# MoHawastaken/Gaussian-Process-Regression

Hardware: AMD Instinct MI355X
Metric: GPR predict-step achieved fp64 TFLOP/s (kernel fill + Cholesky + solves + mean/variance), n x n sqexp (higher is better)
Workload: dtype f64; 1 GPU; c4: n=65536 d=8 sqrexp GPR fit+predict, n*=65536 (reference test-grid rule), noise=0.1; n=65536, d=8, n_star=65536, kernel=sqrexp, parallelism=1-D block-cyclic 512-column panels over 1 GPU(s), test points sliced

## Files before the change

### gaussian-process-regression_amd/_native.py

```python
from __future__ import annotations

import ctypes as C
import os
import threading

import numpy as np

_HERE = os.path.dirname(os.path.abspath(__file__))
LIB_PATH = os.path.join(_HERE, "lib", "libgprc_native" + os.environ.get("GPRC_LIB_SUFFIX", "") + ".so")

CONSTANT, LINEAR, POLYNOMIAL, SQREXP, GAMMAEXP, RATQUAD, SQREXP_ARD, MATERN32, MATERN52, MATERN32_ARD, MATERN52_ARD = range(11)
ARD_KERNELS = (SQREXP_ARD, MATERN32_ARD, MATERN52_ARD)

OK = 0
GPC_REFERENCE_STOP = 1
ERR_ARG, ERR_HIP, ERR_NOMEM, ERR_NOT_PD, ERR_DIVERGED, ERR_MAXITER, ERR_NO_DEVICE = -1, -2, -3, -4, -5, -6, -7


class GprcError(RuntimeError):

    def __init__(self, status: int, message: str):
        super().__init__(f"gprc native error {status}: {message}")
        self.status = status
        self.message = message


class NotPositiveDefinite(ArithmeticError):

    def __init__(self, info: int):
        super().__init__(f"the leading minor of order {info} is not positive definite")
        self.info = info


_dp = C.POINTER(C.c_double)
_i64 = C.c_int64
_vp = C.c_void_p

PROTOTYPES = {
    "gprc_abi_version": (C.c_int, []),
    "gprc_last_error": (C.c_char_p, []),
    "gprc_device_count": (C.c_int, [C.POINTER(C.c_int)]),
    "gprc_ctx_create": (C.c_int, [C.c_int, _vp, C.POINTER(_vp)]),
    "gprc_ctx_destroy": (C.c_int, [_vp]),
    "gprc_ctx_synchronize": (C.c_int, [_vp]),
    "gprc_ctx_trim": (C.c_int, [_vp]),
    "gprc_kernel_matrix": (C.c_int, [_vp, C.c_int, _dp, C.c_int, _vp, _i64, _i64, _vp, _i64, _vp, _i64]),
    "gprc_kernel_colwise": (C.c_int, [_vp, C.c_int, _dp, C.c_int, _vp, _vp, _i64, _i64, _vp]),
    "gprc_gpr_fit": (C.c_int, [_vp, C.c_int, _dp, C.c_int, _vp, _i64, _i64, _vp, C.c_double, C.POINTER(_vp)]),
    "gprc_gpr_fit_retry": (C.c_int, [_vp, C.c_int, _dp, C.c_int, _vp, _i64, _i64, _vp, C.c_double, C.POINTER(_vp),
                                     C.POINTER(C.c_double), C.POINTER(C.c_int)]),
    "gprc_gpr_log_marginal": (C.c_int, [_vp, C.c_int, _dp, C.c_int, _vp, _i64, _i64, _vp, C.c_double, C.POINTER(C.c_double)]),
    "gprc_fit_gradient": (C.c_int, [_vp, C.c_int, _dp, C.c_int, _vp, _i64, _i64, _vp, _dp]),
    "gprc_gpr_logp_grad": (C.c_int, [_vp, C.c_int, _dp, C.c_int, _vp, _i64, _i64, _vp, C.c_double, C.POINTER(C.c_double), _dp]),
    "gprc_gpr_batch_logp_grad": (C.c_int, [_vp, C.c_int, _i64, _vp, C.c_int, _i64, _vp, _vp, _i64, _i64, _i64, _vp, _i64, _vp, _vp, _vp, _vp, _vp]),
    "gprc_gpr_batch_fit": (C.c_int, [_vp, C.c_int, _i64, _vp, C.c_int, _i64, _vp, _vp, _i64, _i64, _i64, _vp, _i64, _vp, C.POINTER(_vp), _vp, _vp]),
    "gprc_gpr_batch_predict": (C.c_int, [_vp, _vp, _i64, _i64, _vp, _vp, _vp, _i64]),
    "gprc_gpr_batch_predict_grad": (C.c_int, [_vp, _vp, _i64, _i64, _vp, _vp, _vp, _i64, _vp, _vp, _i64]),
    "gprc_gpr_batch_loo": (C.c_int, [_vp, _vp, _vp, _vp, _i64, _vp]),
    "gprc_gpr_batch_get_alpha": (C.c_int, [_vp, _vp]),
    "gprc_batch_model_dims": (C.c_int, [_vp, C.POINTER(_i64), C.POINTER(_i64), C.POINTER(_i64)]),
    "gprc_batch_model_free": (C.c_int, [_vp]),
    "gprc_dev_knn": (C.c_int, [_vp, _vp, _i64, _i64, _vp, _i64, _vp, _i64, _vp, _vp, _i64]),
    "gprc_lgpr_create": (C.c_int, [_vp, C.c_int, _dp, C.c_int, _vp, _i64, _i64, _vp, C.c_double, _i64, C.POINTER(_vp)]),
    "gprc_lgpr_set_params": (C.c_int, [_vp, _dp, C.c_int, C.c_double]),
    "gprc_lgpr_predict": (C.c_int, [_vp, _vp, _i64, _vp, _vp, _vp]),
    "gprc_lgpr_neighbours": (C.c_int, [_vp, _vp, _i64, _vp, _vp, _i64]),
    "gprc_lgpr_dims": (C.c_int, [_vp, C.POINTER(_i64), C.POINTER(_i64), C.POINTER(_i64)]),
    "gprc_lgpr_free": (C.c_int, [_vp]),
    "gprc_gpr_loo": (C.c_int, [_vp, _vp, _vp, _vp, C.POINTER(C.c_double)]),
    "gprc_gpr_loo_grad": (C.c_int, [_vp, C.c_int, _dp, C.c_int, _vp, _i64, _i64, _vp, C.c_double, C.POINTER(C.c_double), _dp]),
    "gprc_gpr_predict": (C.c_int, [_vp, _vp, _i64, C.c_int, _vp, _vp]),
    "gprc_gpr_predict_grad": (C.c_int, [_vp, _vp, _i64, _vp, _vp, _vp, _vp]),
    "gprc_gpr_extend": (C.c_int, [_vp, _vp, _i64, _vp]),
    "gprc_model_dims": (C.c_int, [_vp, C.POINTER(_i64), C.POINTER(_i64)]),
    "gprc_model_get_L": (C.c_int, [_vp, _vp, _i64]),
    "gprc_gpr_get_alpha": (C.c_int, [_vp, _vp]),
    "gprc_gpr_get_logp": (C.c_int, [_vp, C.POINTER(C.c_double)]),
    "gprc_gpr_get_noise": (C.c_int, [_vp, C.POINTER(C.c_double)]),
    "gprc_model_free": (C.c_int, [_vp]),
    "gprc_gpc_fit": (C.c_int, [_vp, C.c_int, _dp, C.c_int, _vp, _i64, _i64, _vp, C.c_double, C.c_int, C.c_int, C.POINTER(_vp),
                               C.POINTER(C.c_int)]),
    "gprc_gpc_predict_latent": (C.c_int, [_vp, _vp, _i64, _vp, _vp]),
    "gprc_gpc_predict_class": (C.c_int, [_vp, _vp, _i64, _vp]),
    "gprc_class_probability": (C.c_int, [_vp, _vp, _vp, _i64, _vp]),
    "gprc_gpc_get_f_hat": (C.c_int, [_vp, _vp]),
    "gprc_gpc_get_logq": (C.c_int, [_vp, C.POINTER(C.c_double)]),
    "gprc_gpc_logq_grad": (C.c_int, [_vp, C.c_int, _dp, C.c_int, _vp, _i64, _i64, _vp, C.c_double, C.c_int, C.POINTER(C.c_double), _dp,
                                     C.POINTER(C.c_int)]),
    "gprc_panel_width": (_i64, []),
    "gprc_pad": (_i64, [_i64]),
    "gprc_panel_count": (_i64, [_i64]),
    "gprc_panel_offset": (_i64, [_i64, _i64]),
    "gprc_panel_elems": (_i64, [_i64, _i64]),
    "gprc_packed_size": (_i64, [_i64]),
    "gprc_winv_size": (_i64, [_i64]),
    "gprc_dev_fill_panel": (C.c_int, [_vp, C.c_int, _dp, C.c_int, _vp, _i64, _i64, _i64, C.c_double, _vp, _i64]),
    "gprc_dev_factor_panel": (C.c_int, [_vp, _vp, _i64, _i64, _vp, _vp]),
    "gprc_dev_factor_subpanel": (C.c_int, [_vp, _vp, _i64, _i64, C.c_int, C.c_int, _vp, _vp]),
    "gprc_dev_factor_all": (C.c_int, [_vp, _vp, _i64, _vp, _vp, _vp]),
    "gprc_factor_service": (C.c_int, [C.c_int]),
    "gprc_solve_inv_size": (_i64, [_i64]),
    "gprc_dev_solve_prepare": (C.c_int, [_vp, _vp, _vp, _i64, _vp, _i64, _i64]),
    "gprc_dev_update_trailing": (C.c_int, [_vp, _vp, _i64, _i64, _i64, _i64, _i64]),
    "gprc_dev_update_range": (C.c_int, [_vp, _vp, _i64, _i64, _i64, _i64, _i64, _i64]),
    "gprc_trsv_work_size": (_i64, [_i64]),
    "gprc_dev_trsv": (C.c_int, [_vp, _vp, _vp, _i64, _vp, C.c_int, _vp]),
    "gprc_dev_trsv_step": (C.c_int, [_vp, _vp, _vp, _i64, _vp, C.c_int, _i64, _vp]),
    "gprc_dev_fill_cross": (C.c_int, [_vp, C.c_int, _dp, C.c_int, _vp, _i64, _i64, _i64, _vp, _i64, _i64, _vp, _i64]),
    "gprc_rowreduce_splits": (_i64, [_i64]),
    "gprc_dev_row_reduce": (C.c_int, [_vp, _vp, _i64, _i64, _i64, _vp, _vp, _vp]),
    "gprc_dev_logp": (C.c_int, [_vp, _vp, _i64, _i64, _vp, _vp, _vp]),
    "gprc_gpr_model_from_device": (C.c_int, [_vp, C.c_int, _dp, C.c_int, _vp, _i64, _i64, _vp, _vp, _vp, _vp, C.c_double,
                                             C.c_double, C.POINTER(_vp)]),
    "gprc_mgpu_create": (C.c_int, [C.POINTER(C.c_int), C.c_int, C.c_int, C.POINTER(_vp)]),
    "gprc_mgpu_destroy": (C.c_int, [_vp]),
    "gprc_mgpu_ranks": (C.c_int, [_vp, C.POINTER(C.c_int)]),
    "gprc_mgpu_calibrate": (C.c_int, [_vp, _i64, C.c_int, C.POINTER(C.c_int), C.POINTER(C.c_double)]),
    "gprc_mgpu_exchange_mode": (C.c_int, [_vp, C.POINTER(C.c_int)]),
    "gprc_mgpu_stats": (C.c_int, [_vp, C.POINTER(C.c_double), C.c_int]),
    "gprc_mgpu_gpr_fit": (C.c_int, [_vp, C.c_int, _dp, C.c_int, _vp, _i64, _i64, _vp, C.c_double, C.POINTER(_vp)]),
    "gprc_mgpu_gpr_fit_retry": (C.c_int, [_vp, C.c_int, _dp, C.c_int, _vp, _i64, _i64, _vp, C.c_double, C.POINTER(_vp),
                                          C.POINTER(C.c_double), C.POINTER(C.c_int)]),
    "gprc_mgpu_gpr_predict": (C.c_int, [_vp, _vp, _i64, _vp, _vp]),
    "gprc_mgpu_gpr_get_alpha": (C.c_int, [_vp, _vp]),
    "gprc_mgpu_gpr_get_logp": (C.c_int, [_vp, C.POINTER(C.c_double)]),
    "gprc_mgpu_gpr_get_noise": (C.c_int, [_vp, C.POINTER(C.c_double)]),
    "gprc_mgpu_model_rank": (C.c_int, [_vp, C.c_int, C.POINTER(_vp)]),
    "gprc_mgpu_model_free": (C.c_int, [_vp]),
    "gprc_mvn_factor": (C.c_int, [_vp, _vp, _i64, _i64, C.c_double, _vp, C.POINTER(C.c_int)]),
    "gprc_mvn_sample": (C.c_int, [_vp, _vp, _i64, _i64, _vp, C.c_double, _vp, _i64, _vp, C.POINTER(C.c_int)]),
    "gprc_sym_eigen": (C.c_int, [_vp, _vp, _i64, _i64, _vp, _vp, C.POINTER(C.c_int)]),
    "gprc_combine_all": (C.c_int, [_vp, _vp, C.POINTER(_i64), C.c_int, _vp]),
    "gprc_prof_enable": (C.c_int, [C.c_int]),
    "gprc_prof_panel_trace": (C.c_int, [_vp, C.c_int, C.POINTER(_i64), C.c_int]),
    "gprc_prof_service_trace": (C.c_int, [_vp, C.POINTER(_i64), C.c_int]),
    "gprc_prof_wait_timeout": (C.c_int, [C.POINTER(C.c_int), C.c_int]),
    "gprc_prof_reset": (C.c_int, []),
    "gprc_prof_kinds": (C.c_int, []),
    "gprc_prof_summary": (C.c_int, [C.c_int, C.POINTER(_i64), C.POINTER(C.c_double), C.POINTER(C.c_double), C.POINTER(C.c_double)]),
    "gprc_dev_solve_rows": (C.c_int, [_vp, _vp, _vp, _i64, _vp, _i64, _i64]),
    "gprc_dev_reverse_factor": (C.c_int, [_vp, _vp, _vp, _i64, _vp, _vp]),
    "gprc_sgpr_fit": (C.c_int, [_vp, C.c_int, _dp, C.c_int, _vp, _i64, _i64, _vp, C.c_double, _vp, _i64, C.c_double, C.POINTER(_vp)]),
    "gprc_sgpr_elbo": (C.c_int, [_vp, C.c_int, _dp, C.c_int, _vp, _i64, _i64, _vp, C.c_double, _vp, _i64, C.c_double,
                                 C.POINTER(C.c_double), C.POINTER(C.c_double)]),
    "gprc_sgpr_predict": (C.c_int, [_vp, _vp, _i64, _vp, _vp]),
    "gprc_sgpr_get_elbo": (C.c_int, [_vp, C.POINTER(C.c_double), C.POINTER(C.c_double)]),
    "gprc_sgpr_get_c": (C.c_int, [_vp, _vp]),
    "gprc_dev_gemm_nt": (C.c_int, [_vp, _vp, _i64, _vp, _i64, _vp, _i64, _i64, _i64, _i64, C.c_int]),
    "gprc_dev_gram_rows": (C.c_int, [_vp, _vp, _i64, _i64, _i64, _vp]),
    "gprc_dev_col_reduce": (C.c_int, [_vp, _vp, _i64, _i64, _i64, _vp, _vp]),
    "gprc_sgpr_elbo_grad": (C.c_int, [_vp, C.c_int, _dp, C.c_int, _vp, _i64, _i64, _vp, C.c_double, _vp, _i64, C.c_double,
                                      C.POINTER(C.c_double), _vp, _vp]),
    "gprc_dev_cross_grad": (C.c_int, [_vp, C.c_int, _dp, C.c_int, _vp, _i64, _vp, _i64, _vp, _i64, _i64, C.c_double, _vp, _vp]),
    "gprc_gpr_paths_create": (C.c_int, [_vp, _vp, _vp, _i64, _vp, _vp, _i64, C.POINTER(_vp)]),
    "gprc_gpr_paths_eval": (C.c_int, [_vp, _vp, _i64, _vp, _i64]),
    "gprc_gpr_paths_eval_grad": (C.c_int, [_vp, _vp, _i64, _vp, _i64, _vp, _i64]),
    "gprc_gpr_paths_get_weights": (C.c_int, [_vp, _vp]),
    "gprc_gpr_paths_dims": (C.c_int, [_vp, C.POINTER(_i64), C.POINTER(_i64), C.POINTER(_i64), C.POINTER(_i64)]),
    "gprc_gpr_paths_free": (C.c_int, [_vp]),
    "gprc_dev_feature_gemm": (C.c_int, [_vp, _vp, _vp, _i64, _vp, _i64, _i64, _vp, _i64, _i64, C.c_double, _vp, _i64]),
    "gprc_dev_kernel_gemm": (C.c_int, [_vp, C.c_int, _dp, C.c_int, _vp, _i64, _vp, _i64, _i64, _vp, _i64, _i64, _vp, _i64]),
    "gprc_dev_feature_gemm_grad": (C.c_int, [_vp, _vp, _vp, _i64, _vp, _i64, _i64, _vp, _i64, _i64, C.c_double, _vp, _i64]),
    "gprc_dev_kernel_gemm_grad": (C.c_int, [_vp, C.c_int, _dp, C.c_int, _vp, _i64, _vp, _i64, _i64, _vp, _i64, _i64, _vp, _i64]),
    "gprc_igpr_fit": (C.c_int, [_vp, C.c_int, _dp, C.c_int, _vp, _i64, _i64, _vp, C.c_double, C.c_double, C.c_int, _i64, C.POINTER(_vp)]),
    "gprc_igpr_solve": (C.c_int, [_vp, _vp, _i64, _i64, _vp, _i64, C.POINTER(C.c_int), _dp]),
    "gprc_igpr_predict": (C.c_int, [_vp, _vp, _i64, _vp, _vp]),
    "gprc_igpr_get_alpha": (C.c_int, [_vp, _vp]),
    "gprc_igpr_stats": (C.c_int, [_vp, C.POINTER(C.c_int), C.POINTER(C.c_double), C.POINTER(C.c_double), C.POINTER(_i64)]),
    "gprc_igpr_probes": (C.c_int, [_vp, _vp, _i64, _vp, _i64, _i64, _vp, _i64]),
    "gprc_igpr_logp_grad": (C.c_int, [_vp, _vp, _i64, _vp, _i64, _i64, _dp, _dp, _vp, _vp]),
    "gprc_dev_lowrank_grad": (C.c_int, [_vp, C.c_int, _dp, C.c_int, _vp, _i64, _i64, _vp, _i64, _vp, _i64, _i64, _vp]),
    "gprc_dev_pivoted_cholesky": (C.c_int, [_vp, C.c_int, _dp, C.c_int, _vp, _i64, _i64, _i64, _vp, _i64, _vp, C.POINTER(_i64)]),
}

_lib = None
_lib_lock = threading.Lock()


def _share_hip_runtime_with_torch() -> None:
    import importlib.util
    import sys
    if "torch" in sys.modules:
# ... 124 lines not shown
```

### gaussian-process-regression_amd/csrc/gprc_sched.hip

```cpp
#include <algorithm>
#include <cstdlib>
#include <cstring>

#include "gprc_host.h"

namespace gprc {

static bool panel_steps() {
  static const bool steps = [] { const char* e = std::getenv("GPRC_PANEL"); return e && std::strcmp(e, "steps") == 0; }();
  return steps;
}

int factor_subpanel(gprc_ctx* ctx, double* packed, int64_t n_pad, int64_t p, int j, int part, double* winv, int* info_dev) {
  if (part == 2) return 0;
  hipStream_t s = ctx->stream;
  const int64_t ld = panel_ld(n_pad, p);
  double* pan = packed + panel_offset(n_pad, p);
  const int64_t cj = (int64_t)j * NBI;
  double* wblk = winv + (p * (NB / NBI) + j) * NBI * NBI;
  if (cj > 0)
    GPRC_TRY(launch_gemm_nt(s, pan + cj + cj * ld, ld, pan + cj, ld, pan + cj, ld, ld - cj, NBI, cj, 1, PK_GEMM_INNER));
  GPRC_TRY(launch_potf2_inv(s, pan + cj + cj * ld, ld, wblk, info_dev, (int)(p * NB + cj)));
  const int64_t below = ld - cj - NBI;
  if (below > 0) GPRC_TRY(launch_trsm_panel(s, pan + (cj + NBI) + cj * ld, ld, below, wblk));
  return 0;
}

int factor_panel(gprc_ctx* ctx, double* packed, int64_t n_pad, int64_t p, double* winv, int* info_dev) {
  static const long long trace_p = [] { const char* e = std::getenv("GPRC_PANEL_TRACE"); return e ? std::atoll(e) : -1LL; }();
  static const int trace_mode = std::getenv("GPRC_POTF2_TRACE") != nullptr ? 2 : 1;
  if (!panel_steps()) return launch_panel_fused(ctx->stream, packed, n_pad, p, winv, info_dev, ctx->sync_dev, trace_p == p ? trace_mode : 0);
  for (int j = 0; j < NB / NBI; ++j) GPRC_TRY(factor_subpanel(ctx, packed, n_pad, p, j, 0, winv, info_dev));
  return 0;
}

static int stream_after(gprc_ctx* ctx, hipStream_t to, hipStream_t from) {
  hipEvent_t& ev = ctx->ev_pool[ctx->ev_next++ % 8];
  if (!ev) GPRC_HIP(hipEventCreateWithFlags(&ev, hipEventDisableTiming));
  GPRC_HIP(hipEventRecord(ev, from));
  GPRC_HIP(hipStreamWaitEvent(to, ev, 0));
  return 0;
}

std::atomic<bool> g_service_off{false};

static int64_t want_for(int64_t n_pad) {
  return n_pad < 20480 ? INT64_MAX : 8192;
}

static bool service_carries_inverse(int64_t n_pad) {
  return n_pad < 20480;
}

static bool chain_split(int64_t n_pad) {
  static const int v = [] { const char* e = std::getenv("GPRC_CHAIN_SPLIT"); return e ? std::atoi(e) : -1; }();
  return v >= 0 ? v != 0 : n_pad < 20480;
}

static bool service_shared(int64_t n_pad) {
  static const int v = [] { const char* e = std::getenv("GPRC_SERVICE_SHARE"); return e ? std::atoi(e) : -1; }();
  return n_pad >= 10752 && (v >= 0 ? v != 0 : n_pad >= 13312);
}

static int service_workgroups(bool with_inverse, int64_t n_pad) {
  return SERVICE_CORE_WGS + (with_inverse ? TPP : 0) + (chain_split(n_pad) ? CHAIN_HELPERS : 0);
}

static int launch_group_sweep(gprc_ctx* ctx, double* packed, int64_t n_pad, int64_t g0, int64_t g1, double* winv, int* info_dev, void* sync, void* trace,
                              int service_wgs) {
  int dev = 0, cus = 0;
  GPRC_HIP(hipGetDevice(&dev));
  GPRC_HIP(hipDeviceGetAttribute(&cus, hipDeviceAttributeMultiprocessorCount, dev));
  static const int wgs_env = [] { const char* e = std::getenv("GPRC_SWEEP_WGS"); return e ? std::atoi(e) : 0; }();
  const int per_cu = n_pad < 10752 ? 1 : 2;
  const int shared = service_shared(n_pad) ? service_wgs - 1 - (chain_split(n_pad) ? CHAIN_HELPERS : 0) : 0;
  const int wgs = wgs_env > 0 ? wgs_env : std::max(8, per_cu * (cus - service_wgs) + shared);
  const int core = (per_cu == 1 && wgs_env <= 0) ? 2 : 1;
  static const int head_slices = [] { const char* e = std::getenv("GPRC_HEAD_SLICES"); return e ? std::atoi(e) : 1; }();
  return launch_trailing_sweep(ctx->stream, packed, n_pad, g0, g1, winv, info_dev, sync, trace, wgs, core, core == 2 ? head_slices : 0);
}

static int factor_group_service(gprc_ctx* ctx, double* packed, int64_t n_pad, double* winv, int* info_dev, double* inv, int64_t g0, int64_t g1, void* sync,
                                void* trace, int launches) {
  hipStream_t s = ctx->stream, side = ctx->side_stream;
  GPRC_TRY(stream_after(ctx, side, s));
  const bool shared = service_shared(n_pad), split = chain_split(n_pad);
  if (shared) {
    hipStream_t side2 = ctx->side_stream2;
    GPRC_TRY(stream_after(ctx, side2, s));
    GPRC_TRY(launch_panel_service(side, packed, n_pad, winv, info_dev, sync, trace, service_carries_inverse(n_pad) ? inv : nullptr, g0, g1, split, 1));
    GPRC_TRY(launch_panel_service(side2, packed, n_pad, winv, info_dev, sync, trace, service_carries_inverse(n_pad) ? inv : nullptr, g0, g1, split, 2));
  } else
  GPRC_TRY(launch_panel_service(side, packed, n_pad, winv, info_dev, sync, trace, service_carries_inverse(n_pad) ? inv : nullptr, g0, g1, split, 0));
  static std::atomic<bool> fire{std::getenv("GPRC_TEST_SERVICE_TIMEOUT") != nullptr};
  GPRC_TRY(launch_service_gate(s, n_pad, info_dev, sync, launches, fire.exchange(false)));
  GPRC_TRY(launch_panel_strips(s, packed, n_pad, g0, winv, info_dev, sync, trace));
  static const bool per_panel = [] { const char* e = std::getenv("GPRC_SWEEP"); return e && std::atoi(e) == 0; }();
  if (per_panel) {
    for (int64_t p = g0; p + 1 < g1; ++p) GPRC_TRY(launch_trailing_service(s, packed, n_pad, p, winv, info_dev, sync, trace, g1));
  } else {
    GPRC_TRY(launch_group_sweep(ctx, packed, n_pad, g0, g1, winv, info_dev, sync, trace, service_workgroups(service_carries_inverse(n_pad) && inv, n_pad)));
  }
  GPRC_TRY(stream_after(ctx, s, side));
  if (shared) GPRC_TRY(stream_after(ctx, s, ctx->side_stream2));
  return 0;
}

int factor_all_async(gprc_ctx* ctx, double* packed, int64_t n_pad, double* winv, int* info_dev, double* inv, bool* used_service) {
  hipStream_t s = ctx->stream;
  const int64_t P = n_pad / NB;
  const char* mode = std::getenv("GPRC_FACTOR");
  int64_t want = want_for(n_pad);
  if (mode && std::strcmp(mode, "right") == 0) want = INT64_MAX;
  else if (mode && std::atoll(mode) > 0) want = std::atoll(mode);
  static const int sv_env = [] { const char* e = std::getenv("GPRC_SERVICE"); return e ? std::atoi(e) : -1; }();
  const bool service = !panel_steps() && sv_env != 0 && P >= 2 && !g_service_off.load();
  if (used_service) *used_service = service;
  DevMem sync;
  void* trace = nullptr;
  if (service) {
    if (!ctx->side_stream) {
      int lo = 0, hi = 0;
      GPRC_HIP(hipDeviceGetStreamPriorityRange(&lo, &hi));
      GPRC_HIP(hipStreamCreateWithPriority(&ctx->side_stream, hipStreamNonBlocking, hi));
      GPRC_HIP(hipStreamCreateWithPriority(&ctx->side_stream2, hipStreamNonBlocking, hi));
    }
    GPRC_TRY(sync.alloc((int64_t)(panel_service_sync_bytes(P) + 7) / 8));
    GPRC_HIP(hipMemsetAsync(sync.p, 0, panel_service_sync_bytes(P), s));
    static const bool want_trace = std::getenv("GPRC_SERVICE_TRACE") != nullptr;
    if (want_trace && P <= SVC_TRACE_PANELS) {
      if (!ctx->svc_trace) GPRC_HIP(hipMalloc(&ctx->svc_trace, SVC_TRACE_PANELS * 16 * sizeof(int64_t)));
      GPRC_HIP(hipMemsetAsync(ctx->svc_trace, 0, SVC_TRACE_PANELS * 16 * sizeof(int64_t), s));
      trace = ctx->svc_trace;
    }
  }
  int launches = 0;
  auto sweep = [&]() -> int {
    for (int64_t g0 = 0; g0 < P;) {
      int64_t g1 = g0, tiles = 0;
      while (g1 < P && tiles < want) { tiles += panel_tiles(P, g1); ++g1; }
      GPRC_TRY(launch_trailing_range(s, packed, n_pad, 0, g0, g0, g1, 1));
      if (service) {
        GPRC_TRY(factor_group_service(ctx, packed, n_pad, winv, info_dev, inv, g0, g1, sync.p, trace, ++launches));
      } else {
        for (int64_t p = g0; p < g1; ++p) {
          GPRC_TRY(factor_panel(ctx, packed, n_pad, p, winv, info_dev));
          if (p + 1 < g1) GPRC_TRY(launch_trailing_update(s, packed, n_pad, p, p + 1, g1, 1));
        }
      }
      g0 = g1;
    }
    return (inv && !(service && service_carries_inverse(n_pad))) ? launch_inv512(s, packed, n_pad, winv, inv, 0, P) : 0;
  };
  const int rc = sweep();
  if (rc != 0 && service) {
    (void)hipStreamSynchronize(ctx->side_stream);
    if (ctx->side_stream2) (void)hipStreamSynchronize(ctx->side_stream2);
    (void)hipStreamSynchronize(s);
  }
  return rc;
}


int factor_all(gprc_ctx* ctx, double* packed, int64_t n_pad, double* winv, int* info_host, double* inv, bool* used_service) {
  hipStream_t s = ctx->stream;
  GPRC_HIP(hipMemsetAsync(ctx->info_dev, 0, sizeof(int), s));
  GPRC_TRY(factor_all_async(ctx, packed, n_pad, winv, ctx->info_dev, inv, used_service));
  GPRC_HIP(hipMemcpyAsync(info_host, ctx->info_dev, sizeof(int), hipMemcpyDeviceToHost, s));
  GPRC_HIP(hipStreamSynchronize(s));
  if (*info_host < 0) {
    set_error("factorisation: a device-side dependency wait timed out (info = " + std::to_string(*info_host) + ")" + wait_timeout_report() +
              "; the factor is not valid.  The factor service needs its persistent launch and the caller's kernels to run CONCURRENTLY: "
              "under a tool that serialises dispatches (e.g. rocprofv3 --pmc) set GPRC_SERVICE=0");
    return GPRC_ERR_HIP;
  }
  return 0;
}

int solve_rows(gprc_ctx* ctx, const double* packed, const double* winv, int64_t n_pad, double* vt, int64_t ldv, int64_t m_pad,
               double* sspart, int64_t tri_row0, int64_t p_end) {
  hipStream_t s = ctx->stream;
  const int64_t P = p_end >= 0 ? std::min(p_end, n_pad / NB) : n_pad / NB;
  const char* mode = std::getenv("GPRC_SOLVE");
  int64_t G = (4096 + (m_pad / 128) * (NB / NBI) - 1) / ((m_pad / 128) * (NB / NBI));
  if (mode && std::strcmp(mode, "left") == 0) G = 1;
  else if (mode && std::atoi(mode) > 0) G = std::atoi(mode);
  if ((mode && std::strcmp(mode, "right") == 0) || G > P) G = P;
  auto rows_of = [&](int64_t col_end) {
    if (tri_row0 < 0) return m_pad;
    return std::max<int64_t>(0, std::min<int64_t>(m_pad, pad_up(col_end - tri_row0, 128)));
  };
  for (int64_t g0 = 0; g0 < P; g0 += G) {
    const int64_t g1 = std::min(P, g0 + G);
    const int64_t mg = rows_of(g1 * NB);
    if (mg == 0) continue;
    GPRC_TRY(launch_solve_left(s, vt, ldv, mg, packed, n_pad, g0, g1 - g0, tri_row0));
    static const bool solve_panel_steps = [] { const char* e = std::getenv("GPRC_SOLVE_PANEL"); return e && std::strcmp(e, "steps") == 0; }();
    for (int64_t p = g0; p < g1; ++p) {
      const int64_t ld = panel_ld(n_pad, p);
      const double* pan = packed + panel_offset(n_pad, p);
      const int64_t mp = rows_of((p + 1) * NB);
      if (mp == 0) continue;
      if (!solve_panel_steps) {
        GPRC_TRY(launch_solve_panel_fused(s, vt, ldv, mp, packed, n_pad, p, winv, sspart, m_pad));
      } else
      for (int j = 0; j < NB / NBI; ++j) {
        const int64_t cj = p * NB + (int64_t)j * NBI;
        const double* wblk = winv + (p * (NB / NBI) + j) * NBI * NBI;
        if (j > 0)
          GPRC_TRY(launch_gemm_nt(s, vt + cj * ldv, ldv, vt + p * NB * ldv, ldv, pan + (int64_t)j * NBI, ld, mp, NBI, (int64_t)j * NBI, 0,
                                  PK_GEMM_INNER));
        GPRC_TRY(launch_trsm_panel(s, vt + cj * ldv, ldv, mp, wblk, sspart ? sspart + (cj / NBI) * m_pad : nullptr));
      }
      const int64_t right = (g1 - (p + 1)) * NB;
      if (right > 0)
        GPRC_TRY(launch_gemm_nt(s, vt + (p + 1) * NB * ldv, ldv, vt + p * NB * ldv, ldv, pan + NB, ld, mp, right, NB, 0, PK_SOLVE_UPDATE));
    }
  }
  return 0;
}

bool identity_solve_dense() {
  static const bool dense = std::getenv("GPRC_FITGRAD_DENSE") != nullptr;
  return dense;
}

int64_t predict_partials(int64_t n_pad) { return fill_mean_tiles(n_pad) + n_pad / NBI; }

static int chunk_rows(const gprc_ctx* ctx, int64_t n_pad, int64_t ns) {
  int64_t rows = ((int64_t)(ctx->chunk_bytes / (sizeof(double) * (size_t)n_pad)) - ctx->vt_pad) / 256 * 256;
  if (rows < 256) rows = 256;
  const int64_t need = pad_up(ns, 128);
  return (int)(rows < need ? rows : need);
}

int chunk_workspace(gprc_ctx* ctx, int64_t n_pad, int64_t ns, bool want_tmp, int64_t* rows_out, double** vt, double** part, double** tmp) {
  int64_t rows = chunk_rows(ctx, n_pad, ns);
  const int64_t per_row = (n_pad + predict_partials(n_pad) + 1) * (int64_t)sizeof(double);
  static const bool ignore_meminfo = std::getenv("GPRC_IGNORE_MEMINFO") != nullptr;
  size_t free_b = 0, total_b = 0;
  if (!ignore_meminfo && hipMemGetInfo(&free_b, &total_b) == hipSuccess) {
    int64_t have = 0;
    for (int i = 0; i < 3; ++i) have += ctx->ws_cap[i] * (int64_t)sizeof(double);
    const int64_t avail = (int64_t)free_b + have - ((int64_t)256 << 20);
    const int64_t fit = (avail / per_row - ctx->vt_pad) / 256 * 256;
    if (fit < rows) rows = fit < 256 ? 256 : fit;
  } else {
    (void)hipGetLastError();
  }
  for (;;) {
    const int64_t ldv = rows + ctx->vt_pad;
    int rc = ws_get(ctx, 0, ldv * n_pad, vt);
    if (rc == 0) rc = ws_get(ctx, 1, rows * predict_partials(n_pad), part);
    if (rc == 0 && want_tmp) rc = ws_get(ctx, 2, rows, tmp);
    if (rc == 0) break;
    if (rc != GPRC_ERR_NOMEM || rows <= 256) return rc;
    pool_trim(ctx);
    rows = std::max<int64_t>(256, rows / 2 / 256 * 256);
  }
  *rows_out = rows;
  return 0;
}

}

using namespace gprc;

extern "C" {

int gprc_dev_factor_panel(gprc_ctx* ctx, double* packed, int64_t n_pad, int64_t p, double* winv, int* info_dev) {
  GPRC_TRY(use_device_unless(ctx, n_pad % NB || p < 0 || p >= n_pad / NB || !info_dev, "factor_panel: bad arguments"));
  return factor_panel(ctx, packed, n_pad, p, winv, info_dev);
}

int gprc_dev_factor_subpanel(gprc_ctx* ctx, double* packed, int64_t n_pad, int64_t p, int j, int part, double* winv, int* info_dev) {
  GPRC_TRY(use_device_unless(ctx, n_pad % NB || p < 0 || p >= n_pad / NB || j < 0 || j >= NB / NBI || part < 0 || part > 2 || !info_dev,
                             "factor_subpanel: bad arguments"));
  return factor_subpanel(ctx, packed, n_pad, p, j, part, winv, info_dev);
}
int gprc_dev_factor_all(gprc_ctx* ctx, double* packed, int64_t n_pad, double* winv, int* info_dev, double* inv) {
  GPRC_TRY(use_device_unless(ctx, !packed || !winv || !info_dev || n_pad <= 0 || n_pad % NB, "dev_factor_all: bad arguments"));
  return factor_all_async(ctx, packed, n_pad, winv, info_dev, inv);
}
int gprc_factor_service(int on) {
  const int was = g_service_off.load() ? 0 : 1;
  if (on == 0) g_service_off.store(true);
  else if (on > 0) g_service_off.store(false);
  return was;
}

int gprc_dev_solve_rows(gprc_ctx* ctx, const double* packed, const double* winv, int64_t n_pad, double* vt,
                        int64_t ld, int64_t m_pad) {
  GPRC_TRY(use_device_unless(ctx, m_pad % 128 || n_pad % NB || ld < m_pad || ld % 2, "solve_rows: bad padding"));
  return solve_rows(ctx, packed, winv, n_pad, vt, ld, m_pad);
}

int gprc_dev_reverse_factor(gprc_ctx* ctx, const double* packed, const double* winv, int64_t n_pad, double* packed_rev, double* winv_rev) {
  GPRC_TRY(use_device_unless(ctx, !packed || !winv || !packed_rev || !winv_rev || n_pad <= 0 || n_pad % NB, "dev_reverse_factor: bad arguments"));
  return launch_reverse_factor(ctx->stream, packed, winv, n_pad, packed_rev, winv_rev);
}

int gprc_prof_panel_trace(gprc_ctx* ctx, int side, int64_t* ticks_out, int n) {
  GPRC_TRY(use_device_unless(ctx, !ticks_out || n < 1 || n > 24, "prof_panel_trace: 1..24 stamps"));
  GPRC_HIP(hipDeviceSynchronize());
  GPRC_HIP(hipMemcpy(ticks_out, static_cast<char*>(ctx->sync_dev) + (side ? 256 : 0) + 64, sizeof(int64_t) * (size_t)n, hipMemcpyDeviceToHost));
  return 0;
}

int gprc_prof_service_trace(gprc_ctx* ctx, int64_t* ticks_out, int panels) {
  GPRC_TRY(use_device_unless(ctx, !ticks_out || panels < 1 || panels > SVC_TRACE_PANELS, "prof_service_trace: 1..48 panels"));
  if (!ctx->svc_trace) { set_error("prof_service_trace: no traced sweep on this context (set GPRC_SERVICE_TRACE before the first call)"); return GPRC_ERR_ARG; }
  GPRC_HIP(hipDeviceSynchronize());
  GPRC_HIP(hipMemcpy(ticks_out, ctx->svc_trace, sizeof(int64_t) * 16 * (size_t)panels, hipMemcpyDeviceToHost));
  return 0;
}

int64_t gprc_panel_width(void) { return NB; }
int64_t gprc_pad(int64_t n) { return pad_up(n, NB); }
int64_t gprc_panel_count(int64_t n_pad) { return n_pad / NB; }
int64_t gprc_panel_offset(int64_t n_pad, int64_t p) { return panel_offset(n_pad, p); }
int64_t gprc_panel_elems(int64_t n_pad, int64_t p) { return panel_ld(n_pad, p) * NB; }
int64_t gprc_packed_size(int64_t n_pad) { return panel_offset(n_pad, n_pad / NB); }
int64_t gprc_winv_size(int64_t n_pad) { return n_pad * NBI; }
int64_t gprc_trsv_work_size(int64_t n_pad) { return n_pad + n_pad / NB + 8; }
int64_t gprc_solve_inv_size(int64_t n_pad) { return n_pad * NB; }
int64_t gprc_rowreduce_splits(int64_t cols) { return rowreduce_splits(cols); }

int gprc_dev_fill_panel(gprc_ctx* ctx, int kernel, const double* params_host, int n_params, const double* X,
                        int64_t d, int64_t n, int64_t n_pad, double noise, double* packed, int64_t p) {
  GPRC_TRY(use_device_unless(ctx, n_pad != pad_up(n, NB) || p < 0 || p >= n_pad / NB, "fill_panel: bad layout arguments"));
  KernelSpec ks;
  GPRC_TRY(make_spec(kernel, params_host, n_params, d, &ks));
  return launch_fill(ctx->stream, ks, X, n, X, n, d, packed + panel_offset(n_pad, p), panel_ld(n_pad, p), p * NB, n_pad - p * NB,
                     p * NB, NB, PAD_IDENTITY, noise);
}

int gprc_dev_solve_prepare(gprc_ctx* ctx, const double* packed, const double* winv, int64_t n_pad, double* inv, int64_t p_begin, int64_t p_end) {
  GPRC_TRY(use_device_unless(ctx, !packed || !winv || !inv || n_pad <= 0 || n_pad % NB || p_begin < 0 || p_end > n_pad / NB, "dev_solve_prepare: bad arguments"));
  return launch_inv512(ctx->stream, packed, n_pad, winv, inv, p_begin, p_end);
}
int gprc_dev_update_range(gprc_ctx* ctx, double* packed, int64_t n_pad, int64_t p_begin, int64_t p_end, int64_t q_begin, int64_t q_end,
                          int64_t q_stride) {
  GPRC_TRY(use_device_unless(ctx, !packed || n_pad <= 0 || n_pad % NB || p_begin < 0 || p_end > n_pad / NB, "dev_update_range: bad arguments"));
  if (p_end - p_begin == 1) return launch_trailing_update(ctx->stream, packed, n_pad, p_begin, q_begin, q_end, q_stride);
  return launch_trailing_range(ctx->stream, packed, n_pad, p_begin, p_end, q_begin, q_end, q_stride);
}
int gprc_dev_update_trailing(gprc_ctx* ctx, double* packed, int64_t n_pad, int64_t p, int64_t q_begin,
                             int64_t q_end, int64_t q_stride) {
  GPRC_TRY(use_device_unless(ctx, n_pad % NB, "update_trailing: bad n_pad"));
  if (q_begin >= q_end) return 0;
  return launch_trailing_update(ctx->stream, packed, n_pad, p, q_begin, q_end, q_stride);
}

int gprc_dev_trsv(gprc_ctx* ctx, const double* packed, const double* inv, int64_t n_pad, double* b, int transpose,
                  double* work) {
  GPRC_TRY(use_device_unless(ctx, !packed || !inv || !b || !work || n_pad <= 0 || n_pad % NB, "dev_trsv: bad arguments"));
  return launch_trsv(ctx->stream, packed, inv, n_pad, b, transpose, work);
}

int gprc_dev_trsv_step(gprc_ctx* ctx, const double* packed, const double* inv, int64_t n_pad, double* b, int transpose, int64_t p, double* work) {
  GPRC_TRY(use_device_unless(ctx, !packed || !inv || !b || !work || n_pad <= 0 || n_pad % NB, "dev_trsv_step: bad arguments"));
  return launch_trsv_step(ctx->stream, packed, inv, n_pad, b, transpose, (int)p, work);
}

int gprc_dev_fill_cross(gprc_ctx* ctx, int kernel, const double* params_host, int n_params, const double* X_star,
                        int64_t d, int64_t m, int64_t m_pad, const double* X, int64_t n, int64_t n_pad, double* vt,
// ... 37 lines not shown
```

### include/gprc_native.h

```cpp
#ifndef GPRC_NATIVE_H
#define GPRC_NATIVE_H

#include <stdint.h>

#ifdef __cplusplus
extern "C" {
#endif

#define GPRC_ABI_VERSION 1

#if defined(__GNUC__)
#define GPRC_API __attribute__((visibility("default")))
#else
#define GPRC_API
#endif

typedef enum {
  GPRC_CONSTANT = 0,
  GPRC_LINEAR = 1,
  GPRC_POLYNOMIAL = 2,
  GPRC_SQREXP = 3,
  GPRC_GAMMAEXP = 4,
  GPRC_RATQUAD = 5,
  GPRC_SQREXP_ARD = 6,
// ... 65 lines not shown
typedef struct gprc_local_model gprc_local_model;
GPRC_API int gprc_lgpr_create(gprc_ctx* ctx, int kernel, const double* params, int n_params, const double* X, int64_t d, int64_t n,
                              const double* y, double noise, int64_t m, gprc_local_model** model_out);
GPRC_API int gprc_lgpr_set_params(gprc_local_model* model, const double* params, int n_params, double noise);
GPRC_API int gprc_lgpr_predict(gprc_local_model* model, const double* X_star, int64_t n_star, double* mean_out, double* var_out,
                               int* info_out);
GPRC_API int gprc_lgpr_neighbours(gprc_local_model* model, const double* X_star, int64_t n_star, int* idx_out, double* dist_out,
                                  int64_t ld_out);
GPRC_API int gprc_lgpr_dims(const gprc_local_model* model, int64_t* n_out, int64_t* d_out, int64_t* m_out);
GPRC_API int gprc_lgpr_free(gprc_local_model* model);
GPRC_API int gprc_gpr_loo(gprc_model* model, double* mean_out, double* var_out, double* logdens_out, double* loo_out);
GPRC_API int gprc_gpr_loo_grad(gprc_ctx* ctx, int kernel, const double* params, int n_params, const double* X, int64_t d,
                               int64_t n, const double* y, double noise, double* loo_out, double* grad_out);
GPRC_API int gprc_gpr_predict(gprc_model* model, const double* X_star, int64_t n_star, int pointwise, double* mean_out,
                     double* var_out);
GPRC_API int gprc_gpr_predict_grad(gprc_model* model, const double* X_star, int64_t n_star, double* mean_out, double* var_out,
                                   double* dmean_out, double* dvar_out);
typedef struct gprc_paths gprc_paths;
GPRC_API int gprc_gpr_paths_create(gprc_model* model, const double* Nu, const double* phase, int64_t D, const double* W, const double* E,
                                   int64_t S, gprc_paths** paths_out);
GPRC_API int gprc_gpr_paths_eval(gprc_paths* paths, const double* X_star, int64_t n_star, double* out, int64_t ld_out);
GPRC_API int gprc_gpr_paths_eval_grad(gprc_paths* paths, const double* X_star, int64_t n_star, double* out, int64_t ld_out, double* dout,
                                      int64_t ld_dout);
GPRC_API int gprc_gpr_paths_get_weights(gprc_paths* paths, double* U_out);
GPRC_API int gprc_gpr_paths_dims(const gprc_paths* paths, int64_t* n_out, int64_t* d_out, int64_t* D_out, int64_t* S_out);
GPRC_API int gprc_gpr_paths_free(gprc_paths* paths);
GPRC_API int gprc_gpr_extend(gprc_model* model, const double* X_new, int64_t m, const double* y_new);
GPRC_API int gprc_model_dims(const gprc_model* model, int64_t* n_out, int64_t* d_out);
GPRC_API int gprc_model_get_L(gprc_model* model, double* L_out, int64_t ld_out);
GPRC_API int gprc_gpr_get_alpha(gprc_model* model, double* alpha_out);
GPRC_API int gprc_gpr_get_logp(gprc_model* model, double* logp_out);
GPRC_API int gprc_gpr_get_noise(gprc_model* model, double* noise_out);
GPRC_API int gprc_model_free(gprc_model* model);

GPRC_API int gprc_sgpr_fit(gprc_ctx* ctx, int kernel, const double* params, int n_params, const double* X, int64_t d, int64_t n,
                           const double* y, double noise, const double* Z, int64_t m, double jitter, gprc_model** model_out);
GPRC_API int gprc_sgpr_elbo(gprc_ctx* ctx, int kernel, const double* params, int n_params, const double* X, int64_t d, int64_t n,
                            const double* y, double noise, const double* Z, int64_t m, double jitter, double* elbo_out, double* trace_out);
GPRC_API int gprc_sgpr_elbo_grad(gprc_ctx* ctx, int kernel, const double* params, int n_params, const double* X, int64_t d, int64_t n,
                                 const double* y, double noise, const double* Z, int64_t m, double jitter, double* elbo_out,
                                 double* grad_out, double* dZ_out);
GPRC_API int gprc_sgpr_predict(gprc_model* model, const double* X_star, int64_t n_star, double* mean_out, double* var_out);
GPRC_API int gprc_sgpr_get_elbo(gprc_model* model, double* elbo_out, double* trace_out );
GPRC_API int gprc_sgpr_get_c(gprc_model* model, double* c_out);

GPRC_API int gprc_igpr_fit(gprc_ctx* ctx, int kernel, const double* params, int n_params, const double* X, int64_t d, int64_t n,
                           const double* y, double noise, double tol, int max_iter, int64_t precond_rank, gprc_model** model_out);
GPRC_API int gprc_igpr_solve(gprc_model* model, const double* B, int64_t ldb, int64_t S, double* Xout, int64_t ldx, int* iters_out,
                             double* relres_true_out);
GPRC_API int gprc_igpr_predict(gprc_model* model, const double* X_star, int64_t n_star, double* mean, double* var);
GPRC_API int gprc_igpr_get_alpha(gprc_model* model, double* alpha_out);
GPRC_API int gprc_igpr_stats(gprc_model* model, int* iterations_out, double* relres_recurrence_out, double* relres_true_out, int64_t* rank_out);
GPRC_API int gprc_igpr_probes(gprc_model* model, const double* G1, int64_t ldg1, const double* G2, int64_t ldg2, int64_t T, double* Z_out,
                              int64_t ldz);
GPRC_API int gprc_igpr_logp_grad(gprc_model* model, const double* G1, int64_t ldg1, const double* G2, int64_t ldg2, int64_t T, double* logp_out,
                                 double* se_out, double* grad_out, double* terms_out);

#define GPRC_GPC_REFERENCE_STOP 1
GPRC_API int gprc_gpc_fit(gprc_ctx* ctx, int kernel, const double* params, int n_params, const double* X, int64_t d,
                 int64_t n, const double* y, double epsilon, int max_iter, int flags, gprc_model** model_out,
                 int* iters_out);
GPRC_API int gprc_gpc_predict_latent(gprc_model* model, const double* X_star, int64_t n_star, double* fs_bar_out,
                            double* Vfs_out);
GPRC_API int gprc_gpc_predict_class(gprc_model* model, const double* X_star, int64_t n_star, double* prob_out);
GPRC_API int gprc_class_probability(gprc_ctx* ctx, const double* fs_bar, const double* Vfs, int64_t n, double* prob_out);
GPRC_API int gprc_gpc_get_f_hat(gprc_model* model, double* f_hat_out);
GPRC_API int gprc_gpc_get_logq(gprc_model* model, double* logq_out);
GPRC_API int gprc_gpc_logq_grad(gprc_ctx* ctx, int kernel, const double* params, int n_params, const double* X, int64_t d, int64_t n,
                                const double* y, double epsilon, int max_iter, double* logq_out, double* grad_out, int* iters_out);

GPRC_API int64_t gprc_panel_width(void);
GPRC_API int64_t gprc_pad(int64_t n);
GPRC_API int64_t gprc_panel_count(int64_t n_pad);
GPRC_API int64_t gprc_panel_offset(int64_t n_pad, int64_t p);
GPRC_API int64_t gprc_panel_elems(int64_t n_pad, int64_t p);
GPRC_API int64_t gprc_packed_size(int64_t n_pad);
GPRC_API int64_t gprc_winv_size(int64_t n_pad);
GPRC_API int gprc_dev_fill_panel(gprc_ctx* ctx, int kernel, const double* params_host, int n_params, const double* X,
                        int64_t d, int64_t n, int64_t n_pad, double noise, double* packed, int64_t p);
GPRC_API int gprc_dev_factor_panel(gprc_ctx* ctx, double* packed, int64_t n_pad, int64_t p, double* winv, int* info_dev);
GPRC_API int gprc_dev_factor_subpanel(gprc_ctx* ctx, double* packed, int64_t n_pad, int64_t p, int j, int part, double* winv,
                             int* info_dev);
GPRC_API int gprc_dev_factor_all(gprc_ctx* ctx, double* packed, int64_t n_pad, double* winv, int* info_dev, double* inv);
GPRC_API int gprc_factor_service(int on);
#define GPRC_INFO_WAIT_TIMEOUT (-99)
GPRC_API int gprc_dev_update_trailing(gprc_ctx* ctx, double* packed, int64_t n_pad, int64_t p, int64_t q_begin,
                             int64_t q_end, int64_t q_stride);
GPRC_API int gprc_dev_update_range(gprc_ctx* ctx, double* packed, int64_t n_pad, int64_t p_begin, int64_t p_end, int64_t q_begin,
                          int64_t q_end, int64_t q_stride);
GPRC_API int64_t gprc_solve_inv_size(int64_t n_pad);
GPRC_API int gprc_dev_solve_prepare(gprc_ctx* ctx, const double* packed, const double* winv, int64_t n_pad, double* inv, int64_t p_begin,
                           int64_t p_end);
GPRC_API int64_t gprc_trsv_work_size(int64_t n_pad);
GPRC_API int gprc_dev_trsv(gprc_ctx* ctx, const double* packed, const double* inv, int64_t n_pad, double* b, int transpose,
                  double* work);
GPRC_API int gprc_dev_trsv_step(gprc_ctx* ctx, const double* packed, const double* inv, int64_t n_pad, double* b, int transpose,
                       int64_t p, double* work);
GPRC_API int gprc_dev_fill_cross(gprc_ctx* ctx, int kernel, const double* params_host, int n_params, const double* X_star,
                        int64_t d, int64_t m, int64_t m_pad, const double* X, int64_t n, int64_t n_pad, double* vt,
                        int64_t ld);
GPRC_API int64_t gprc_rowreduce_splits(int64_t cols);
GPRC_API int gprc_dev_row_reduce(gprc_ctx* ctx, const double* vt, int64_t ld, int64_t rows, int64_t cols, const double* w,
                        double* out, double* work);
GPRC_API int gprc_dev_logp(gprc_ctx* ctx, const double* packed, int64_t n_pad, int64_t n, const double* y, const double* alpha,
                  double* out_dev);
GPRC_API int gprc_gpr_model_from_device(gprc_ctx* ctx, int kernel, const double* params, int n_params, const double* X,
                               int64_t d, int64_t n, const double* y, double* packed, double* winv, double* alpha,
                               double noise, double logp, gprc_model** model_out);
GPRC_API int gprc_dev_solve_rows(gprc_ctx* ctx, const double* packed, const double* winv, int64_t n_pad, double* vt,
                        int64_t ld, int64_t m_pad);
GPRC_API int gprc_dev_reverse_factor(gprc_ctx* ctx, const double* packed, const double* winv, int64_t n_pad, double* packed_rev,
                                     double* winv_rev);
GPRC_API int gprc_dev_gemm_nt(gprc_ctx* ctx, double* C, int64_t ldc, const double* A, int64_t lda, const double* B, int64_t ldb, int64_t M,
                              int64_t N, int64_t K, int lower);
GPRC_API int gprc_dev_gram_rows(gprc_ctx* ctx, const double* vt, int64_t ld, int64_t rows, int64_t n_pad, double* packed);
GPRC_API int gprc_dev_col_reduce(gprc_ctx* ctx, const double* vt, int64_t ld, int64_t rows, int64_t cols, const double* w, double* out);
GPRC_API int gprc_dev_cross_grad(gprc_ctx* ctx, int kernel, const double* params, int n_params, const double* G, int64_t ld, const double* A,
                                 int64_t rows, const double* Z, int64_t cols, int64_t d, double f, double* grad_out, double* dZ);
GPRC_API int gprc_dev_feature_gemm(gprc_ctx* ctx, const double* Nu, const double* phase, int64_t D, const double* A, int64_t rows, int64_t d,
                                   const double* W, int64_t ldw, int64_t S, double scale, double* out, int64_t ld);
GPRC_API int gprc_dev_kernel_gemm(gprc_ctx* ctx, int kernel, const double* params, int n_params, const double* A, int64_t rows,
                                  const double* Bpts, int64_t cols, int64_t d, const double* U, int64_t ldu, int64_t S, double* out, int64_t ld);
GPRC_API int gprc_dev_feature_gemm_grad(gprc_ctx* ctx, const double* Nu, const double* phase, int64_t D, const double* A, int64_t rows, int64_t d,
                                        const double* W, int64_t ldw, int64_t S, double scale, double* dout, int64_t ld);
GPRC_API int gprc_dev_kernel_gemm_grad(gprc_ctx* ctx, int kernel, const double* params, int n_params, const double* A, int64_t rows,
                                       const double* Bpts, int64_t cols, int64_t d, const double* U, int64_t ldu, int64_t S, double* dout, int64_t ld);
GPRC_API int gprc_dev_lowrank_grad(gprc_ctx* ctx, int kernel, const double* params, int n_params, const double* X, int64_t d, int64_t n,
                                   const double* A, int64_t lda, const double* B, int64_t ldb, int64_t R, double* grad_out);
GPRC_API int gprc_dev_pivoted_cholesky(gprc_ctx* ctx, int kernel, const double* params, int n_params, const double* X, int64_t d, int64_t n,
                                       int64_t r, double* L, int64_t ldl, int64_t* piv_out, int64_t* rank_out);

#define GPRC_MGPU_RCCL 1
#define GPRC_MGPU_NO_LOOKAHEAD 2
#define GPRC_MGPU_SCATTER_ALLGATHER 4
#define GPRC_MGPU_AUTO_EXCHANGE 8
typedef struct gprc_mgpu gprc_mgpu;
typedef struct gprc_mgpu_model gprc_mgpu_model;
GPRC_API int gprc_mgpu_create(const int* devices, int n_ranks, int flags, gprc_mgpu** mgpu_out);
GPRC_API int gprc_mgpu_destroy(gprc_mgpu* mgpu);
GPRC_API int gprc_mgpu_ranks(const gprc_mgpu* mgpu, int* n_ranks_out);
GPRC_API int gprc_mgpu_calibrate(gprc_mgpu* mgpu, int64_t doubles, int reps, int* choice_out, double* ms_out);
GPRC_API int gprc_mgpu_exchange_mode(const gprc_mgpu* mgpu, int* mode_out);
GPRC_API int gprc_mgpu_stats(const gprc_mgpu* mgpu, double* out, int n);
GPRC_API int gprc_mgpu_gpr_fit(gprc_mgpu* mgpu, int kernel, const double* params, int n_params, const double* X, int64_t d,
                      int64_t n, const double* y, double noise, gprc_mgpu_model** model_out);
GPRC_API int gprc_mgpu_gpr_fit_retry(gprc_mgpu* mgpu, int kernel, const double* params, int n_params, const double* X, int64_t d,
                            int64_t n, const double* y, double noise, gprc_mgpu_model** model_out, double* noise_used,
                            int* attempts);
GPRC_API int gprc_mgpu_gpr_predict(gprc_mgpu_model* model, const double* X_star, int64_t n_star, double* mean_out,
                          double* var_out);
GPRC_API int gprc_mgpu_gpr_get_alpha(gprc_mgpu_model* model, double* alpha_out);
GPRC_API int gprc_mgpu_gpr_get_logp(gprc_mgpu_model* model, double* logp_out);
GPRC_API int gprc_mgpu_gpr_get_noise(gprc_mgpu_model* model, double* noise_out);
GPRC_API int gprc_mgpu_model_rank(gprc_mgpu_model* model, int rank, gprc_model** model_out);
GPRC_API int gprc_mgpu_model_free(gprc_mgpu_model* model);

GPRC_API int gprc_mvn_factor(gprc_ctx* ctx, const double* cov, int64_t ld, int64_t m, double tol, double* L_out, int* method_out);
GPRC_API int gprc_mvn_sample(gprc_ctx* ctx, const double* cov, int64_t ld, int64_t m, const double* mean, double tol, const double* Z,
                    int64_t n_draws, double* out, int* method_out);
GPRC_API int gprc_sym_eigen(gprc_ctx* ctx, const double* A, int64_t lda, int64_t m, double* values_out, double* vectors_out,
                   int* sweeps_out);

GPRC_API int gprc_combine_all(gprc_ctx* ctx, const double* axis_values, const int64_t* lengths, int d, double* out);
GPRC_API int gprc_prof_enable(int on);
GPRC_API int gprc_prof_panel_trace(gprc_ctx* ctx, int side, int64_t* ticks_out, int n);
GPRC_API int gprc_prof_service_trace(gprc_ctx* ctx, int64_t* ticks_out, int panels);
// ... 10 lines not shown
```

Baseline: 75.07 TFLOP/s.

## Plan Cholesky panel group boundaries with a cost-model dynamic program

```diff
diff --git a/gaussian-process-regression_amd/_native.py b/gaussian-process-regression_amd/_native.py
--- a/gaussian-process-regression_amd/_native.py
+++ b/gaussian-process-regression_amd/_native.py
@@ -98,6 +98,7 @@
     "gprc_dev_factor_panel": (C.c_int, [_vp, _vp, _i64, _i64, _vp, _vp]),
     "gprc_dev_factor_subpanel": (C.c_int, [_vp, _vp, _i64, _i64, C.c_int, C.c_int, _vp, _vp]),
     "gprc_dev_factor_all": (C.c_int, [_vp, _vp, _i64, _vp, _vp, _vp]),
+    "gprc_dev_plan_groups": (C.c_int, [_i64, C.c_int, _vp, C.c_int]),
     "gprc_factor_service": (C.c_int, [C.c_int]),
     "gprc_solve_inv_size": (_i64, [_i64]),
     "gprc_dev_solve_prepare": (C.c_int, [_vp, _vp, _vp, _i64, _vp, _i64, _i64]),
diff --git a/gaussian-process-regression_amd/csrc/gprc_sched.hip b/gaussian-process-regression_amd/csrc/gprc_sched.hip
--- a/gaussian-process-regression_amd/csrc/gprc_sched.hip
+++ b/gaussian-process-regression_amd/csrc/gprc_sched.hip
@@ -1,8 +1,10 @@
 #include <algorithm>
 #include <cstdlib>
 #include <cstring>
+#include <vector>
 
 #include "gprc_host.h"
+#include "host_plan.h"
 
 namespace gprc {
 
@@ -44,8 +46,18 @@
 
 std::atomic<bool> g_service_off{false};
 
-static int64_t want_for(int64_t n_pad) {
-  return n_pad < 20480 ? INT64_MAX : 8192;
+static bool planned_from(int64_t n_pad) {
+  return n_pad >= 20480;
+}
+
+static int plan_slots(int* slots) {
+  static const int env = [] { const char* e = std::getenv("GPRC_PLAN_SLOTS"); return e ? std::atoi(e) : 0; }();
+  if (env > 0) { *slots = env; return 0; }
+  int dev = 0, cus = 0;
+  GPRC_HIP(hipGetDevice(&dev));
+  GPRC_HIP(hipDeviceGetAttribute(&cus, hipDeviceAttributeMultiprocessorCount, dev));
+  *slots = 2 * cus;
+  return 0;
 }
 
 static bool service_carries_inverse(int64_t n_pad) {
@@ -110,9 +122,14 @@
   hipStream_t s = ctx->stream;
   const int64_t P = n_pad / NB;
   const char* mode = std::getenv("GPRC_FACTOR");
-  int64_t want = want_for(n_pad);
-  if (mode && std::strcmp(mode, "right") == 0) want = INT64_MAX;
-  else if (mode && std::atoll(mode) > 0) want = std::atoll(mode);
+  std::vector<int> bounds;
+  if (mode && std::strcmp(mode, "right") == 0) bounds = plan_constant(P, TPP, INT64_MAX);
+  else if (mode && std::atoll(mode) > 0) bounds = plan_constant(P, TPP, std::atoll(mode));
+  else if (planned_from(n_pad) || (mode && std::strcmp(mode, "plan") == 0)) {
+    int slots = 0;
+    GPRC_TRY(plan_slots(&slots));
+    bounds = plan_groups(PLAN_MODEL_MI355X, P, TPP, slots);
+  } else bounds = plan_constant(P, TPP, INT64_MAX);
   static const int sv_env = [] { const char* e = std::getenv("GPRC_SERVICE"); return e ? std::atoi(e) : -1; }();
   const bool service = !panel_steps() && sv_env != 0 && P >= 2 && !g_service_off.load();
   if (used_service) *used_service = service;
@@ -136,9 +153,9 @@
   }
   int launches = 0;
   auto sweep = [&]() -> int {
+    auto cut = bounds.begin();
     for (int64_t g0 = 0; g0 < P;) {
-      int64_t g1 = g0, tiles = 0;
-      while (g1 < P && tiles < want) { tiles += panel_tiles(P, g1); ++g1; }
+      const int64_t g1 = *++cut;
       GPRC_TRY(launch_trailing_range(s, packed, n_pad, 0, g0, g0, g1, 1));
       if (service) {
         GPRC_TRY(factor_group_service(ctx, packed, n_pad, winv, info_dev, inv, g0, g1, sync.p, trace, ++launches));
@@ -282,6 +299,13 @@
   GPRC_TRY(use_device_unless(ctx, !packed || !winv || !info_dev || n_pad <= 0 || n_pad % NB, "dev_factor_all: bad arguments"));
   return factor_all_async(ctx, packed, n_pad, winv, info_dev, inv);
 }
+int gprc_dev_plan_groups(int64_t n_pad, int slots, int* bounds, int cap) {
+  if (n_pad <= 0 || n_pad % NB || slots < 1 || !bounds) { set_error("dev_plan_groups: bad arguments"); return GPRC_ERR_ARG; }
+  const std::vector<int> b = plan_groups(PLAN_MODEL_MI355X, n_pad / NB, TPP, slots);
+  if ((int64_t)b.size() > cap) { set_error("dev_plan_groups: " + std::to_string(b.size()) + " boundaries do not fit in cap"); return GPRC_ERR_ARG; }
+  std::copy(b.begin(), b.end(), bounds);
+  return (int)b.size() - 1;
+}
 int gprc_factor_service(int on) {
   const int was = g_service_off.load() ? 0 : 1;
   if (on == 0) g_service_off.store(true);
diff --git a/gaussian-process-regression_amd/csrc/host_plan.h b/gaussian-process-regression_amd/csrc/host_plan.h
--- /dev/null
+++ b/gaussian-process-regression_amd/csrc/host_plan.h
@@ -0,0 +1,81 @@
+#pragma once
+#include <stdint.h>
+
+#include <vector>
+
+namespace gprc {
+
+struct PlanModel {
+  double pass_launch;
+  double tile_fixed;
+  double tile_per_panel;
+  double group_fixed;
+  double group_per_panel;
+  double group_per_strip;
+  double group_per_update;
+};
+constexpr PlanModel PLAN_MODEL_MI355X = {0.3587, 0.0, 0.11127, 0.1021, 0.1708, 0.000619, 0.12310};
+
+constexpr int PLAN_MIN_GROUP = 2;
+constexpr int PLAN_MAX_GROUP = 40;
+
+inline int64_t plan_panel_tiles(int64_t P, int64_t tpp, int64_t q) { return tpp * tpp * (P - q) - tpp * (tpp - 1) / 2; }
+
+inline int64_t plan_pass_tiles(int64_t P, int64_t tpp, int64_t g0, int64_t g1) {
+  int64_t t = 0;
+  for (int64_t q = g0; q < g1; ++q) t += plan_panel_tiles(P, tpp, q);
+  return t;
+}
+
+inline double plan_group_cost(const PlanModel& m, int64_t P, int64_t tpp, int64_t slots, int64_t g0, int64_t g1) {
+  double ms = 0.0;
+  if (g0 > 0) {
+    const int64_t per_cu = slots / 2 > 0 ? slots / 2 : 1;
+    const int64_t halves = (plan_pass_tiles(P, tpp, g0, g1) + per_cu - 1) / per_cu;
+    ms += m.pass_launch + 0.5 * (double)halves * (m.tile_fixed + m.tile_per_panel * (double)g0);
+  }
+  int64_t strips = 0, updates = 0;
+  for (int64_t q = g0; q < g1; ++q) {
+    strips += (P - q) * tpp;
+    updates += (q - g0) * plan_panel_tiles(P, tpp, q);
+  }
+  return ms + m.group_fixed + m.group_per_panel * (double)(g1 - g0) + m.group_per_strip * (double)strips +
+         m.group_per_update * (double)updates / (double)slots;
+}
+
+inline double plan_cost(const PlanModel& m, int64_t P, int64_t tpp, int64_t slots, const int* bounds, int groups) {
+  double ms = 0.0;
+  for (int g = 0; g < groups; ++g) ms += plan_group_cost(m, P, tpp, slots, bounds[g], bounds[g + 1]);
+  return ms;
+}
+
+inline std::vector<int> plan_constant(int64_t P, int64_t tpp, int64_t want) {
+  std::vector<int> bounds{0};
+  for (int64_t g0 = 0; g0 < P;) {
+    int64_t g1 = g0, tiles = 0;
+    while (g1 < P && tiles < want) { tiles += plan_panel_tiles(P, tpp, g1); ++g1; }
+    bounds.push_back((int)g1);
+    g0 = g1;
+  }
+  return bounds;
+}
+
+inline std::vector<int> plan_groups(const PlanModel& m, int64_t P, int64_t tpp, int64_t slots) {
+  if (P < PLAN_MIN_GROUP || slots < 1) return {0, (int)P};
+  const double inf = 1e300;
+  std::vector<double> f((size_t)P + 1, inf);
+  std::vector<int> from((size_t)P + 1, -1);
+  f[0] = 0.0;
+  for (int64_t j = PLAN_MIN_GROUP; j <= P; ++j)
+    for (int64_t i = j - PLAN_MAX_GROUP < 0 ? 0 : j - PLAN_MAX_GROUP; i + PLAN_MIN_GROUP <= j; ++i) {
+      if (f[(size_t)i] >= inf) continue;
+      const double c = f[(size_t)i] + plan_group_cost(m, P, tpp, slots, i, j);
+      if (c < f[(size_t)j]) { f[(size_t)j] = c; from[(size_t)j] = (int)i; }
+    }
+  std::vector<int> rev;
+  for (int j = (int)P; j > 0; j = from[(size_t)j]) rev.push_back(j);
+  rev.push_back(0);
+  return std::vector<int>(rev.rbegin(), rev.rend());
+}
+
+}
diff --git a/include/gprc_native.h b/include/gprc_native.h
--- a/include/gprc_native.h
+++ b/include/gprc_native.h
@@ -171,6 +171,7 @@
 GPRC_API int gprc_dev_factor_subpanel(gprc_ctx* ctx, double* packed, int64_t n_pad, int64_t p, int j, int part, double* winv,
                              int* info_dev);
 GPRC_API int gprc_dev_factor_all(gprc_ctx* ctx, double* packed, int64_t n_pad, double* winv, int* info_dev, double* inv);
+GPRC_API int gprc_dev_plan_groups(int64_t n_pad, int slots, int* bounds, int cap);
 GPRC_API int gprc_factor_service(int on);
 #define GPRC_INFO_WAIT_TIMEOUT (-99)
 GPRC_API int gprc_dev_update_trailing(gprc_ctx* ctx, double* packed, int64_t n_pad, int64_t p, int64_t q_begin,
```

Result: no change. 75.32 TFLOP/s, median of 6 (+0.3%).
